# tprelle/janusgraph

Measured on AMD Instinct MI355X. Metric: GTEPS for PageRank iter + BFS, RMAT-24/26, 1/2/4/8 GPUs; % of HBM peak, higher is better.
Workload: dtype f64

## Files before the change

### janusgraph_amd/csrc/jg_api.cpp

```cpp
#include <dlfcn.h>
#include <execinfo.h>

#include <algorithm>
#include <atomic>
#include <cstdlib>
#include <cstring>
#include <limits>
#include <map>
#include <mutex>

#include "jg_cache.h"
#include "jg_internal.h"
#include "jg_labelset.h"

namespace jg {

namespace {
thread_local std::string g_last_error;
}

void rccl_check(ncclResult_t r, const char* what) {
    if (r != ncclSuccess) fail(JG_ERR_RCCL, std::string(what) + ": " + ncclGetErrorString(r));
}

// ... 625 lines not shown
    if (!(cond)) jg::fail(JG_ERR_ARG, msg)

extern "C" {

int jg_abi_version(void) { return JG_ABI_VERSION; }

int jg_tune_set(const char* key, int64_t value) {
    JG_GUARD_BEGIN
    JG_ARG(key, "null key");
    const std::string k(key);
    jg::Tune& t = jg::tune();
    if (k == "dev_poison_probe") {
        jg::dev_poison_probe(value);
        return JG_OK;
    }
    struct Knob {
        const char* name;
        int* field;
        int64_t lo, hi;
    };
    const Knob knobs[] = {
        {"pull_split", &t.pull_split, 0, 1},
        {"halo", &t.halo, 0, 1},
        {"bfs_alpha", &t.bfs_alpha, 1, 1000000},
        {"dobfs_alpha", &t.dobfs_alpha, 1, 1000000},
        {"bfs_beta", &t.bfs_beta, 1, 1000000},
        {"bfs_narrow", &t.bfs_narrow, 0, 1},
        {"nb_alpha", &t.nb_alpha, 1, 1000000},
        {"nb_first", &t.nb_first, 4, 4096},
        {"cc_push", &t.cc_push, 0, 1},
        {"msbfs_sparse", &t.msbfs_sparse, 0, 1},
        {"msbfs_td", &t.msbfs_td, 0, 2},
        {"cc_first", &t.cc_first, 1, 64},
        {"msbfs_skip", &t.msbfs_skip, 0, 1},
        {"msbfs_exit", &t.msbfs_exit, 0, 2},
        {"msbfs_td_rowapply", &t.msbfs_td_rowapply, 0, 1024},
        {"msbfs_td_noprobe", &t.msbfs_td_noprobe, 0, 1000},
        {"msbfs_scan_queue", &t.msbfs_scan_queue, 0, 1001},
        {"msbfs_exit_first", &t.msbfs_exit_first, 1, 256},
        {"msbfs_exit_live", &t.msbfs_exit_live, 0, 1000},
        {"cc_uf", &t.cc_uf, 0, 1},
        {"cc_uf_sharded", &t.cc_uf_sharded, 0, 1},
        {"cc_uf_search", &t.cc_uf_search, 0, 1},
        {"cc_sparse", &t.cc_sparse, 0, 1},
        {"msbfs_split", &t.msbfs_split, 0, 1},
        {"sharded_bfs", &t.sharded_bfs, 0, 1},
        {"bfs_td_split", &t.bfs_td_split, 0, 2},
        {"bfs_td_split_levels", &t.bfs_td_split_levels, 0, 0xffff},
        {"bfs_batch0", &t.bfs_batch0, 1, 64},
        {"bfs_grid_mult", &t.bfs_grid_mult, 1, 64},
        {"bfs_grid", &t.bfs_grid, 64, 65536},
        {"bfs_tail_grid", &t.bfs_tail_grid, 0, 65536},
        {"merge_temporal", &t.merge_temporal, 0, 2},
        {"sd_delta", &t.sd_delta, -1, 1 << 30},
        {"sd_dist32", &t.sd_dist32, 0, 2},
    };
    for (const Knob& kn : knobs) {
        if (k != kn.name) continue;
        if (value < kn.lo || value > kn.hi)
            jg::fail(JG_ERR_ARG, k + " must be in [" + std::to_string(kn.lo) + ", " + std::to_string(kn.hi) + "]");
        *kn.field = (int)value;
        return JG_OK;
    }
    if (k.rfind("band", 0) == 0 && k.size() == 9 && k[4] >= '0' && k[4] <= '3' &&
        (k.substr(5) == "_deg" || k.substr(5) == "_bit" || k.substr(5) == "_sub")) {
        const int i = k[4] - '0';
        if (k.substr(5) == "_deg") {
            JG_ARG(value >= -1, "band degree must be >= 0 (0: unused) or -1 (automatic)");
            t.band_deg[i] = value;
        } else if (k.substr(5) == "_bit") {
            JG_ARG(value == 0 || (value >= 3 && value <= 8), "band bits must be 0 (automatic) or in [3, 8]");
            t.band_bits[i] = value == 0 ? -1 : (int)value;
        } else {
            JG_ARG(value >= 1 && value <= 256 && (value & (value - 1)) == 0, "band sub-slices must be a power of two in [1, 256]");
            int b = 0;
            while ((1 << b) < value) ++b;
            t.band_bits[i] = b;
        }
    } else if (k.size() == 12 && k.compare(0, 11, "merge_stage") == 0 && k[11] >= '0' && k[11] <= '3') {
        JG_ARG(value == -1 || value == 0 || value == 64 || value == 128 || value == 256 || value == 512,
               "merge_stage<i> must be -1 (automatic), 0, 64, 128, 256 or 512");
        t.merge_stage[k[11] - '0'] = (int)value;
    } else if (k == "bfs_td_split_min" || k == "bfs_td_split_max") {
        JG_ARG(value >= 1 && value <= INT32_MAX, "bfs_td_split_min / _max must be in [1, 2^31)");
        (k == "bfs_td_split_min" ? t.bfs_td_split_min : t.bfs_td_split_max) = value;
    } else if (k == "merge_pack") {
        JG_ARG(value == 0 || value == 1 || value == 24, "merge_pack must be 0 (32 bits), 1 (automatic) or 24 (at least 24)");
        t.merge_pack = (int)value;
    } else if (k == "pull_unroll" || k == "pull_nt" || k == "pull_lds" || k == "light_lds" || k == "slice_lds" ||
               k == "pull_short" || k == "pull_overlap" || k == "bfs_persistent") {
    } else {
        jg::fail(JG_ERR_ARG, "unknown tuning key: " + k);
    }
    JG_GUARD_END
}

const char* jg_last_error(void) { return jg::g_last_error.c_str(); }

int jg_comm_unique_id(void* out) {
    JG_GUARD_BEGIN
    JG_ARG(out, "null output");
    ncclUniqueId id;
    jg::rccl_check(ncclGetUniqueId(&id), "ncclGetUniqueId");
    static_assert(sizeof(ncclUniqueId) == JG_UNIQUE_ID_BYTES, "unique id size");
    std::memcpy(out, &id, sizeof id);
    JG_GUARD_END
// ... 834 lines not shown
```

### janusgraph_amd/csrc/jg_internal.h

```cpp
#pragma once

#include <algorithm>
#include <memory>
#include <atomic>
#include <mutex>
#include <functional>
#include <vector>

#include "jg_common.h"
#include "janusgpu.h"

#include <rccl/rccl.h>

namespace jg {

struct Csr {
    int64_t rows = 0;
    int64_t nnz = 0;
    DevBuf<int64_t> row_ptr;
    DevBuf<int32_t> col;
    DevBuf<int32_t> weight;
    mutable int64_t empty_from = -1;
    mutable DevBuf<int32_t> first_col;
    mutable long long wstat[4] = {0, 0, 0, 0};
// ... 68 lines not shown
    return (x ^ (x >> 8) ^ (x >> 16) ^ (x >> 24)) & 255u;
}
__host__ __device__ __forceinline__ uint32_t brev_bits(uint32_t v, int bits) {
    uint32_t r = 0;
    for (int i = 0; i < bits; ++i) r |= ((v >> i) & 1u) << (bits - 1 - i);
    return r;
}
__host__ __device__ __forceinline__ uint32_t sub_key(int64_t c) { return brev_bits(sub_hash(c), 8); }
__host__ __device__ __forceinline__ int sub_slice(int64_t c, int bits) { return (int)(sub_hash(c) & ((1u << bits) - 1)); }

struct Ctx;

struct CompactMap {
    const uint32_t* bits = nullptr;
    const int64_t* off = nullptr;
    const int64_t* qbase = nullptr;
    int64_t S = 0;
    int r = 0, tbits = 31;
    __host__ __device__ bool on() const { return bits != nullptr; }
    __device__ __forceinline__ int32_t operator()(int64_t g) const {
        const int64_t q = g / S, l = g - q * S;
        if (q == r) return (int32_t)l;
        const uint32_t w = bits[g >> 5];
        const int64_t rank = off[g >> 5] + __popc(w & ((1u << (g & 31)) - 1u)) - qbase[q];
        return (int32_t)(((q < r ? q + 1 : q) << tbits) + rank);
    }
};

struct Halo {
    bool on = false;
    int tbits = 31;
    int64_t C = 0;
    DevBuf<uint32_t> bits;
    DevBuf<int64_t> off, qbase;
    DevBuf<int32_t> send_src;
    std::vector<int64_t> send_off, recv_off;
    DevBuf<uint64_t> send_buf;
    int seg_of(int q, int r) const { return q < r ? q + 1 : q; }
    CompactMap map(int64_t S, int r) const {
        CompactMap m;
        if (on) { m.bits = bits.get(); m.off = off.get(); m.qbase = qbase.get(); m.S = S; m.r = r; m.tbits = tbits; }
        return m;
    }
};

struct alignas(16) IdSlot {
    unsigned long long key;
    uint32_t val, pad;
};

struct VecPos {
    int64_t base = 0;
    __device__ __forceinline__ int64_t operator()(int64_t row) const { return base + row; }
};

struct Shard {
    int device = 0;
    int index = 0;
    int vtag = -1;
    hipStream_t stream = nullptr;
    ncclComm_t comm = nullptr;
    int64_t rows = 0;
    Csr in, out, both;
    PullPlan plan_in, plan_both;
    PullPlan plan_out;
    bool plan_out_built = false;
    Halo halo_in, halo_both;
    DevBuf<int32_t> out_degree;
    mutable std::vector<int32_t> dense_of_local_host;
    mutable std::mutex lazy_mu;
    const std::vector<int32_t>& dense_of_local() const;
    DevBuf<int32_t> dense_rows;

    DevBuf<double> pr_contrib[2];
    DevBuf<double> pr_rank;
    DevBuf<double> pr_hub_partial;
    DevBuf<double> pr_split_partial;
    DevBuf<int32_t> cc_split_partial;
    DevBuf<int32_t> cc_msg[2];
    DevBuf<int32_t> cc_label;
    DevBuf<int32_t> cc_rank0;
    DevBuf<int32_t> cc_depth;
    DevBuf<unsigned long long> cc_linked;
    int64_t cc_heavy = -1;
    DevBuf<int32_t> cc_hub_partial;
    DevBuf<int32_t> cc_changed;
    DevBuf<int32_t> bfs_queue[2];
    DevBuf<int64_t> bfs_qoff[2];
    DevBuf<unsigned long long> bfs_bm[2];
    DevBuf<uint8_t> bfs_seen;
    DevBuf<int32_t> bfs_owner;
    DevBuf<unsigned long long> bfs_ctr;
    DevBuf<unsigned char> bfs_state;
    DevBuf<int32_t> bfs_depth;
    bool bfs_depth_tail_clean = false;
    DevBuf<uint8_t> sbfs_stamp;
    DevBuf<uint8_t> sbfs_dirty;
    DevBuf<unsigned long long> sbfs_bq;
    DevBuf<int32_t> sbfs_bpre;
    bool sbfs_stamp_clean = false;
    int bfs_hist[4] = {0, 0, 0, 0};
    int bfs_hist_n = 0;
    int sd_hist[4] = {0, 0, 0, 0};
    int sd_hist_n = 0;
    DevBuf<int32_t> kept_depth;
    DevBuf<int32_t> dag_vertex, dag_depth, dag_pred;
    DevBuf<int64_t> dag_off;
    DevBuf<int64_t> census_vid, census_pop;
    std::vector<DevBuf<uint8_t>> nb_level;
    DevBuf<uint8_t> nb_vis;
    DevBuf<unsigned long long> nb_rest;
    DevBuf<int32_t> nb_queue[2];
    DevBuf<int64_t> nb_qoff[2];
    DevBuf<unsigned long long> nb_ctr;
    DevBuf<unsigned char> nb_state;
    DevBuf<const uint8_t*> nb_table;

    std::vector<hipEvent_t> prof_events;
    std::vector<hipEvent_t> exch_events;
    std::vector<int> prof_units;
};

inline bool same_device(const Shard& sh, int dev) { return sh.device == dev && sh.vtag <= 0; }

struct Graph {
    Ctx* ctx = nullptr;
    int64_t n = 0;
    int P = 1;
    int64_t S = 0;
    uint32_t flags = 0;
    std::vector<std::unique_ptr<Shard>> shards;
    DevBuf<IdSlot> id_table;
    int id_dev = 0;
    std::vector<int64_t> vid;
    DevBuf<int32_t> padded_dev;
    mutable std::vector<int32_t> padded_host;
    mutable std::mutex lazy_mu;
    const std::vector<int32_t>& padded_of_dense() const;
    jg_graph_info info{};
    bool has_weights = false;
    int kept_nsrc = 0;
    int kept_dir = 0;
    int64_t dag_nv = -1, dag_ne = 0;
    int64_t census_listed = -1;
    int64_t top_listed = -1;
    std::vector<int64_t> top_index;
    std::vector<double> top_rank, top_edges;
    bool cc_ranks = false;
    DevBuf<int64_t> cc_vor;
    mutable std::vector<int64_t> cc_vor_host;
    const std::vector<int64_t>& vid_of_rank() const;
    int pr_cur = 0;
    bool pr_begun = false;
    double pr_damping = 0.85;
    int64_t pr_vertex_count = 1;
    int pr_steps = 0;

    int64_t vid_of(int64_t dense) const { return vid.empty() ? dense : vid[dense]; }
    int64_t padded_len() const { return (int64_t)P * S; }
    const Halo& halo(const Shard& sh, uint32_t adj) const { return adj == JG_ADJ_BOTH ? sh.halo_both : sh.halo_in; }
    int64_t vec_len(const Shard& sh, uint32_t adj) const {
        const Halo& h = halo(sh, adj);
        return h.on ? std::max<int64_t>(h.C, 1) : padded_len();
    }
    VecPos vec_pos(const Shard& sh, uint32_t adj) const {
        VecPos p;
        p.base = halo(sh, adj).on ? 0 : (int64_t)sh.index * S;
        return p;
    }
};

struct Ctx {
    std::vector<int> devices;
    int nranks = 1;
    int rank = 0;
    bool logical = false;
    bool vdev = false;
    std::vector<ncclComm_t> comms;
    bool host_transport = false;
    jg_transport transport{};
    std::vector<hipStream_t> streams;
    bool profiling = false;
    jg_stats last{};
    std::atomic<int> live{0};
    int total_shards() const { return nranks * (int)devices.size(); }
};

struct DenseEdges {
    std::vector<int32_t*> src, dst;
    std::vector<int32_t*> weight;
    int64_t m = 0;
    bool capped = false, in_from_in = false;
    std::vector<int32_t*> out_src, in_src, in_dst;
    int64_t m_in = 0;
    int64_t truncated_rows = 0;
};
void build_graph_from_dense(Graph& g, DenseEdges& e);
void generate_rmat_device(int scale, uint64_t seed, int64_t m, int32_t* src, int32_t* dst, hipStream_t s);
void remap_ids_device(const int64_t* d_vid, int64_t n, const int64_t* d_src, const int64_t* d_dst, int64_t m,
                      int32_t* dsrc, int32_t* ddst, hipStream_t s, DevBuf<IdSlot>* table = nullptr);
void dense_of_vids(const Graph& g, const int64_t* vids, int64_t k, int64_t* out, int64_t* padded = nullptr);
void mask_ids_device(const int64_t* masked, const int32_t* dense, int64_t m, int32_t* out, hipStream_t s);
void build_pull_plan(Shard& sh, const Csr& csr, PullPlan& plan, int64_t col_space, int64_t vec_entries,
                     int elem_bytes);
int auto_band_bits(int64_t vec_entries, int elem_bytes);

void rccl_check(ncclResult_t r, const char* what);

void exchange_vec(Graph& g, uint32_t adj, std::vector<void*>& bufs, size_t elem_bytes, ncclDataType_t type);
// ... 156 lines not shown
};
NarrowRun narrow_bfs(Ctx& ctx, Shard& sh, const Csr& push, const Csr& pull, const int64_t* src, int ns, int max_depth,
                     int32_t* planes);
void combine_run(Graph& g, int direction, int combiner, int wrap32, const int64_t* init, int steps, int64_t* out,
                 uint8_t* received_out);

int allreduce_or(Graph& g, int flag);
void allreduce_sum_i64(Graph& g, int64_t* vals, int n);
uint64_t allreduce_or_u64(Graph& g, uint64_t v);

bool pull_split_launches();
bool debug_plan();
bool debug_bfs();

struct Tune {
    int pull_split = 1;
    int64_t band_deg[4] = {96, -1, -1, 0};
    int band_bits[4] = {-1, -1, -1, 3};
    int halo = 1;
    int bfs_alpha = 14;
    int dobfs_alpha = 30;
    int bfs_beta = 24;
    int bfs_narrow = 1;
    int nb_alpha = 30;
    int nb_first = 16;
    int cc_push = 1;
    int msbfs_sparse = 1;
    int msbfs_td = 1;
    int cc_first = 1;
    int msbfs_skip = 1;
    int msbfs_exit = 1;
    int msbfs_td_rowapply = 4;
    int msbfs_td_noprobe = 2;
    int msbfs_scan_queue = 50;
    int msbfs_exit_first = 16;
    int msbfs_exit_live = 950;
    int cc_uf = 1;
    int cc_uf_sharded = 1;
    int cc_uf_search = 1;
    int cc_sparse = 1;
    int msbfs_split = 1;
    int sharded_bfs = 1;
    int bfs_td_split = 2;
    int bfs_td_split_levels = 2;
    int64_t bfs_td_split_min = 65536;
    int64_t bfs_td_split_max = 1 << 20;
    int bfs_batch0 = 10;
    int bfs_grid_mult = 4;
    int bfs_grid = 8192;
    int bfs_tail_grid = 64;
    int sd_dist32 = 1;
    int sd_delta = -1;
    int merge_temporal = 1;
    int merge_stage[4] = {-1, -1, -1, -1};
    int merge_pack = 1;
};
Tune& tune();
void host_allgather(Ctx& c, const void* in, void* out, size_t bytes);
void host_exchange(Ctx& c, const std::vector<int>& speer, const std::vector<const void*>& sbuf,
                   const std::vector<size_t>& sbytes, const std::vector<int>& rpeer, const std::vector<void*>& rbuf,
                   const std::vector<size_t>& rbytes);
int device_cu_count();

bool prof_enabled(const Ctx& c);
void prof_record_start(Ctx& c, Shard& sh);
void prof_record_stop(Ctx& c, Shard& sh, int units = 1);
void prof_collect(Ctx& c, Graph& g);
void exch_record(Ctx& c, Shard& sh);
void prof_discard_exchanges(Graph& g);
struct ExchTimer {
    Graph& g;
    explicit ExchTimer(Graph& gr);
    ~ExchTimer();
};

}

struct jg_ctx {
    jg::Ctx impl;
};
struct jg_graph {
    jg::Graph impl;
    explicit jg_graph(jg::Ctx* c) {
        impl.ctx = c;
        c->live.fetch_add(1);
    }
    ~jg_graph() { impl.ctx->live.fetch_sub(1); }
    jg_graph(const jg_graph&) = delete;
    jg_graph& operator=(const jg_graph&) = delete;
};
```

### janusgraph_amd/csrc/jg_pagerank.hip

```cpp
#include <cstdlib>

#include "jg_pull.h"
#include "jg_scatter.h"

namespace jg {

namespace {

struct PrOp {
    using T = double;
    const double* __restrict__ x;
    double* __restrict__ contrib_out;
    double* __restrict__ rank;
    const int32_t* __restrict__ outdeg;
    VecPos pos;
    double damping, teleport;
    bool write_rank;
    __device__ __forceinline__ double identity() const { return 0.0; }
    __device__ __forceinline__ double combine(double a, double b) const { return __dadd_rn(a, b); }
    __device__ __forceinline__ double gather(int32_t c) const { return x[c]; }
    __device__ __forceinline__ const double* vec() const { return x; }
    __device__ __forceinline__ double shfl_xor(double v, int o) const { return __shfl_xor(v, o, kWave); }
    __device__ __forceinline__ bool active(int64_t) const { return true; }
    __device__ __forceinline__ void finalize(int64_t row, double s) const {
        const double r = __dadd_rn(__dmul_rn(damping, s), teleport);
        if (write_rank) rank[row] = r;
        contrib_out[pos(row)] = r / (double)outdeg[row];
    }
};

__global__ void pr_init_kernel(const int32_t* __restrict__ outdeg, int64_t rows, VecPos pos, double initial,
                               double* __restrict__ contrib, double* __restrict__ rank) {
    for (int64_t l = (int64_t)blockIdx.x * blockDim.x + threadIdx.x; l < rows; l += (int64_t)gridDim.x * blockDim.x) {
        rank[l] = initial;
        contrib[pos(l)] = initial / (double)outdeg[l];
    }
}

void exchange_contrib(Graph& g, int which) {
    std::vector<void*> bufs;
    for (auto& sp : g.shards) bufs.push_back(sp->pr_contrib[which].peer());
    exchange_vec(g, JG_ADJ_IN, bufs, sizeof(double), ncclFloat64);
}

}

void pagerank_begin(Graph& g, double damping, int64_t vertex_count) {
    if (!(g.flags & JG_ADJ_IN)) fail(JG_ERR_UNSUPPORTED, "PageRank needs a graph built with JG_ADJ_IN");
    if (vertex_count == 0) fail(JG_ERR_ARG, "vertexCount must be non-zero");
    for (auto& sp : g.shards) {
        Shard& sh = *sp;
        DeviceGuard dg(sh);
        const int64_t len = g.vec_len(sh, JG_ADJ_IN);
        for (int k = 0; k < 2; ++k) {
            if (sh.pr_contrib[k].size() != (size_t)len) sh.pr_contrib[k].alloc(len);
            JG_HIP(hipMemsetAsync(sh.pr_contrib[k].get(), 0, sh.pr_contrib[k].bytes(), sh.stream));
        }
        if (sh.pr_rank.size() != (size_t)std::max<int64_t>(sh.rows, 1)) {
            const char* f = std::getenv("JG_VDEV_FAULT");
            if (f && *f && *f != '0' && sh.index > 0) {
                DeviceGuard d0(*g.shards[0]);
                sh.pr_rank.alloc(std::max<int64_t>(sh.rows, 1));
            } else {
                sh.pr_rank.alloc(std::max<int64_t>(sh.rows, 1));
            }
        }
        if (sh.pr_hub_partial.size() != (size_t)std::max<int64_t>(sh.plan_in.num_chunks, 1))
            sh.pr_hub_partial.alloc(std::max<int64_t>(sh.plan_in.num_chunks, 1));
        if (sh.pr_split_partial.size() != (size_t)sh.plan_in.split_partial_len()) {
            sh.pr_split_partial.alloc(sh.plan_in.split_partial_len());
        }
        const double initial = 1.0 / (double)vertex_count;
        if (sh.rows > 0) {
            pr_init_kernel<<<grid_for(sh.rows), kBlock, 0, sh.stream>>>(sh.out_degree.get(), sh.rows,
                                                                        g.vec_pos(sh, JG_ADJ_IN), initial,
                                                                        sh.pr_contrib[0].get(), sh.pr_rank.get());
            JG_LAUNCH_CHECK();
        }
    }
    exchange_contrib(g, 0);
    g.pr_cur = 0;
    g.pr_begun = true;
    g.pr_damping = damping;
    g.pr_vertex_count = vertex_count;
    g.pr_steps = 0;
}

void pagerank_steps(Graph& g, int nsteps) {
    if (!g.pr_begun) fail(JG_ERR_STATE, "jg_pagerank_step before jg_pagerank_begin");
    const double teleport = (1.0 - g.pr_damping) / (double)g.pr_vertex_count;
    Ctx* pc = g.ctx->profiling ? g.ctx : nullptr;
    Shard* whole = (pc && g.shards.size() == 1 && g.ctx->total_shards() == 1 && nsteps > 0) ? g.shards[0].get() : nullptr;
    if (whole) {
        DeviceGuard dg(whole->device);
        prof_record_start(*pc, *whole);
        pc = nullptr;
    }
    for (int t = 0; t < nsteps; ++t) {
        const int cur = g.pr_cur, nxt = cur ^ 1;
        for (auto& sp : g.shards) {
            Shard& sh = *sp;
            DeviceGuard dg(sh);
            PrOp op;
            op.x = sh.pr_contrib[cur].get();
            op.contrib_out = sh.pr_contrib[nxt].get();
            op.rank = sh.pr_rank.get();
            op.outdeg = sh.out_degree.get();
            op.pos = g.vec_pos(sh, JG_ADJ_IN);
            op.damping = g.pr_damping;
            op.teleport = teleport;
            op.write_rank = t == nsteps - 1 || g.pr_steps < 2;
            const bool skip_empty = g.pr_steps >= 2;
            launch_pull(sh.in, sh.plan_in, op, sh.pr_hub_partial.get(), sh.stream, pc, &sh, sh.pr_split_partial.get(),
                        skip_empty);
        }
        exchange_contrib(g, nxt);
        g.pr_cur = nxt;
        ++g.pr_steps;
    }
    if (whole) {
        DeviceGuard dg(whole->device);
        prof_record_stop(*g.ctx, *whole, nsteps);
    }
}

void pagerank_end(Graph& g, double* rank_out, double* edge_count_out) {
    if (!g.pr_begun) fail(JG_ERR_STATE, "jg_pagerank_end before jg_pagerank_begin");
    for (auto& sp : g.shards) {
        Shard& sh = *sp;
        DeviceGuard dg(sh);
        JG_HIP(hipStreamSynchronize(sh.stream));
        if (sh.rows == 0) continue;
        if (rank_out) rows_to_dense(g, sh, sh.pr_rank.get(), rank_out);
        if (edge_count_out) rows_to_dense(g, sh, sh.out_degree.get(), edge_count_out);
    }
    prof_collect(*g.ctx, g);
}

}
```

### janusgraph_amd/csrc/jg_pull.h

```cpp
#pragma once

#include <type_traits>

#include "jg_internal.h"
#include "jg_prim.h"

namespace jg {

struct PullArgs {
    const int64_t* __restrict__ row_ptr;
    const int32_t* __restrict__ col;
    const int64_t* __restrict__ chunk_row;
    const int64_t* __restrict__ chunk_begin;
    const int64_t* __restrict__ chunk_end;
    const int64_t* __restrict__ hub_chunk_ptr;
    int64_t num_chunks;
    int64_t num_hub_rows;
    int64_t class_row_begin[kNumClasses];
    int64_t class_row_end[kNumClasses];
    int64_t class_block_begin[kNumClasses + 1];
    int64_t block_offset;
    int64_t skip_rows;
    int runs;
    int64_t run_begin[kRunMax + 1];
// ... 177 lines not shown
            T t = red[0];
#pragma unroll
            for (int w = 1; w < kBlock / kWave; ++w) t = op.combine(t, red[w]);
            hub_partial[b] = t;
        }
        return;
    }
    pull_block_rows<Op, U>(a, op, GlobalGather<Op>{op}, b, (int)threadIdx.x);
}

template <class Op, int U>
__global__ __launch_bounds__(kBlock) void pull_kernel(PullArgs a, Op op, typename Op::T* __restrict__ hub_partial) {
    pull_block<Op, U>(a, op, hub_partial, (int64_t)blockIdx.x + a.block_offset);
}

template <class Op>
__global__ void pull_hub_finalize_kernel(PullArgs a, Op op, const typename Op::T* __restrict__ hub_partial) {
    using T = typename Op::T;
    for (int64_t h = (int64_t)blockIdx.x * blockDim.x + threadIdx.x; h < a.num_hub_rows;
         h += (int64_t)gridDim.x * blockDim.x) {
        const int64_t c0 = a.hub_chunk_ptr[h], c1 = a.hub_chunk_ptr[h + 1];
        if (a.chunk_row[c0] < a.skip_rows) continue;
        T acc = op.identity();
        for (int64_t k = c0; k < c1; ++k) acc = op.combine(acc, hub_partial[k]);
        op.finalize(a.chunk_row[c0], acc);
    }
}

constexpr int kMergeThreads = 1024;
constexpr int kMergeWaves = kMergeThreads / kWave;
constexpr int kMergeEpl = kMergeTask / kWave;
constexpr int kMergeLdsBytes = 160 * 1024;

struct MergeArgs {
    const uint4* __restrict__ pack_a;
    const uint32_t* __restrict__ pack_b;
    const uint8_t* __restrict__ heads;
    const int32_t* __restrict__ meta;
    const int64_t* __restrict__ sub_begin;
    const int64_t* __restrict__ sub_end;
    const int64_t* __restrict__ sub_base;
    int64_t tasks;
    int bits;
    int stage;
    const uint32_t* __restrict__ live;
};

struct HotSegs {
    int32_t hs = 0;
    int tbits = 31;
    int nseg = 1;
};

template <class Op, bool MSEG = true>
struct SliceGather {
    using T = typename Op::T;
    const Op& op;
    lds_ptr<const T> lds;
    uint32_t hg;
    int sb;
    int bits;
    uint32_t hmask, h;
    uint32_t idcell;
    __device__ __forceinline__ bool is_hot(uint32_t loc) const {
        if constexpr (!MSEG) return loc < (hg << 4);
        return ((loc >> 4) & ((1u << sb) - 1u)) < hg;
    }
    __device__ __forceinline__ T hot(uint32_t loc, bool valid) const {
        if constexpr (!MSEG) return lds[valid && loc < (hg << 4) ? loc : idcell];
        const uint32_t g = loc >> 4, j = g & ((1u << sb) - 1u), seg = g >> sb;
        return lds[valid && j < hg ? (((seg * hg + j) << 4) | (loc & 15u)) : idcell];
    }
    __device__ __forceinline__ int32_t col(uint32_t loc) const {
        const uint32_t x = (loc >> 4) << bits;
        const uint32_t hx = (x ^ (x >> 8) ^ (x >> 16) ^ (x >> 24)) & hmask;
        return (int32_t)(((x | (h ^ hx)) << 4) | (loc & 15u));
    }
    __device__ __forceinline__ T cold(uint32_t loc, bool valid, bool lds_on) const {
        T v = op.identity();
        if (valid && !(lds_on && is_hot(loc))) v = op.gather(col(loc));
        return v;
    }
};

template <int W>
__device__ __forceinline__ uint32_t unpack_entry(const uint32_t (&d)[W / 4], int u) {
    const int o = W * u, i = o >> 5, sh = o & 31;
    uint32_t v = d[i] >> sh;
    if (sh + W > 32) v |= d[i + 1] << (32 - sh);
    if constexpr (W < 32) v &= (1u << W) - 1u;
    return v;
}

template <class T>
__device__ __forceinline__ T lane_up(T v, int lane, int d) {
    static_assert(sizeof(T) % 4 == 0, "whole dwords");
    int w[sizeof(T) / 4];
    __builtin_memcpy(w, &v, sizeof(T));
    const int addr = ((lane - d) & (kWave - 1)) << 2;
#pragma unroll
    for (size_t i = 0; i < sizeof(T) / 4; ++i) w[i] = __builtin_amdgcn_ds_bpermute(addr, w[i]);
    __builtin_memcpy(&v, w, sizeof(T));
    return v;
}

template <class Op, class = void>
struct op_task_live : std::false_type {};
template <class Op>
struct op_task_live<Op, std::void_t<decltype(Op::kTaskLive)>> : std::bool_constant<Op::kTaskLive> {};

template <class Op, bool LDS, int PW, bool MSEG = false>
__global__ __launch_bounds__(kMergeThreads) void pull_merge_kernel(MergeArgs a, Op op, typename Op::T* __restrict__ partial,
                                                                   typename Op::T* __restrict__ carry, HotSegs hs,
                                                                   int temporal) {
    using T = typename Op::T;
    extern __shared__ __align__(16) unsigned char merge_lds[];
    const int S = 1 << a.bits;
    const int xs = S < kXcds ? S : kXcds;
    const int rep = kXcds / xs;
    const int per = S / xs;
    const int w = (int)(blockIdx.x >> 3), W = (int)(gridDim.x >> 3);
    const int xcd = (int)(blockIdx.x & (kXcds - 1));
    const int wave = threadIdx.x / kWave, lane = threadIdx.x % kWave;
    lds_ptr<T> hotv = (lds_ptr<T>)merge_lds;
    const int gshift = 4 + a.bits;
    const int hg = hs.hs >> gshift;
    const int nl = hs.nseg * hg;
    lds_ptr<T> stg = hotv + (nl * 16 + 1) + wave * (a.stage + 1);
    lds_ptr<uint32_t> tctr = (lds_ptr<uint32_t>)(hotv + (nl * 16 + 1) + kMergeWaves * (a.stage + 1));
    const int rounds = temporal ? per : 1;
    const uint32_t hmask = (1u << a.bits) - 1u;
    auto image_line = [&](int seg, int j, int hh) {
        const int64_t grp = ((int64_t)seg << (hs.tbits - gshift)) + j;
        return (grp << a.bits) + (int64_t)(hh ^ (sub_hash(grp << gshift) & hmask));
    };
    for (int rd = 0; rd < rounds; ++rd) {
    const int h = (xcd % xs) | ((temporal ? rd : w % per) << 3);
    const int64_t g = (int64_t)(temporal ? w : w / per) * rep + xcd / xs;
    const int64_t G = (int64_t)(temporal ? W : W / per) * rep;
    if constexpr (LDS) {
        if (rd > 0) __syncthreads();
        constexpr int kStage = 8;
        constexpr int kUnit = 16 / (int)sizeof(T);
        static_assert(16 % sizeof(T) == 0 && kUnit <= 16, "16-byte staging units");
        const unsigned char* src = reinterpret_cast<const unsigned char*>(op.vec());
        const int units = nl * 16 / kUnit;
        using u4 = uint32_t __attribute__((ext_vector_type(4)));
        lds_ptr<u4> hv4 = (lds_ptr<u4>)merge_lds;
        for (int q0 = 0; q0 < units; q0 += kStage * kMergeThreads) {
            u4 buf[kStage];
#pragma unroll
            for (int u = 0; u < kStage; ++u) {
                const int q = q0 + u * kMergeThreads + (int)threadIdx.x;
                const int i = q * kUnit, sg = i >> 4;
                int seg = 0, j = sg;
                if (hs.nseg > 1) {
                    seg = sg / hg;
                    j = sg - seg * hg;
                }
                buf[u] = u4{0, 0, 0, 0};
                if (q < units)
                    buf[u] = *reinterpret_cast<const u4*>(src + (image_line(seg, j, h) * 16 + (i & 15)) * (int64_t)sizeof(T));
            }
#pragma unroll
            for (int u = 0; u < kStage; ++u) {
                const int q = q0 + u * kMergeThreads + (int)threadIdx.x;
                if (q < units) hv4[q] = buf[u];
            }
        }
        if (threadIdx.x == 0) {
            hotv[nl * 16] = op.identity();
            *tctr = 0u;
        }
        __syncthreads();
    }
    const SliceGather<Op, MSEG> lg{op,       hotv, (uint32_t)hg, hs.tbits - gshift, a.bits, (1u << a.bits) - 1u, (uint32_t)h,
                             (uint32_t)nl * 16u};
    const int64_t base = a.sub_base[h];
    const int64_t ntask = a.sub_base[h + 1] - base;
    const int64_t hbegin = a.sub_begin[h], hend = a.sub_end[h];
    constexpr bool dyn = LDS;
    const int64_t grot = (g + rd) % G;
    auto task_of = [&](int64_t j) { return j * G + grot; };
    auto grab = [&]() -> int64_t {
        uint32_t j = 0;
        if (lane == 0) j = __hip_atomic_fetch_add(tctr, 1u, __ATOMIC_RELAXED, __HIP_MEMORY_SCOPE_WORKGROUP);
        return task_of((int64_t)__builtin_amdgcn_readfirstlane(j));
    };
    int64_t jstat = wave;
    auto advance = [&]() -> int64_t {
        if (dyn) return grab();
        jstat += kMergeWaves;
        return task_of(jstat);
    };
    auto dead = [&](int64_t kk) -> bool {
        if constexpr (!op_task_live<Op>::value) return false;
        if (a.live == nullptr || kk >= ntask) return false;
        const uint64_t tt = (uint64_t)(base + kk);
        const uint32_t wd = __builtin_amdgcn_readfirstlane(a.live[tt >> 5]);
        return ((wd >> (tt & 31)) & 1u) == 0;
    };
    int64_t k = dyn ? grab() : task_of(jstat);
    while (dead(k)) k = advance();
    if (k >= ntask) continue;
    static_assert(kMergeEpl == 8, "a lane chunk is 8 entries");
    constexpr int DB = PW / 4 - 4;
    auto chunk = [&](int64_t kk) { return (hbegin >> 3) + kk * kWave + lane; };
    auto meta_idx = [&](int64_t kk) { return 2 * (base + kk) + (lane & 1); };
    auto head_idx = [&](int64_t kk) { return (base + kk) * kWave + lane; };
    auto ld = [](const auto* p) { return *p; };
    using v4u = uint32_t __attribute__((ext_vector_type(4)));
    using v2u = uint32_t __attribute__((ext_vector_type(2)));
    auto load_chunk = [&](int64_t kk, uint32_t (&d)[PW / 4]) {
        const int64_t x = chunk(kk);
        const v4u va = ld(reinterpret_cast<const v4u*>(a.pack_a) + x);
        d[0] = va.x, d[1] = va.y, d[2] = va.z, d[3] = va.w;
        if constexpr (DB == 1) {
            d[4] = ld(a.pack_b + x);
        } else if constexpr (DB == 2) {
            const v2u vb = ld(reinterpret_cast<const v2u*>(a.pack_b) + x);
            d[4] = vb.x, d[5] = vb.y;
        } else {
            const v4u vb = ld(reinterpret_cast<const v4u*>(a.pack_b) + x);
            d[4] = vb.x, d[5] = vb.y, d[6] = vb.z, d[7] = vb.w;
        }
    };
    uint32_t cd[PW / 4];
    load_chunk(k, cd);
    uint32_t hb = ld(a.heads + head_idx(k));
    int32_t mw = ld(a.meta + meta_idx(k));
// ... 211 lines not shown
}

template <class Op>
__global__ void pull_slice_finalize_kernel(int64_t row0, int64_t rows, Op op, FinalizeBands fb,
                                           const typename Op::T* __restrict__ partial) {
    for (int64_t r = row0 + (int64_t)blockIdx.x * blockDim.x + threadIdx.x; r < rows; r += (int64_t)gridDim.x * blockDim.x)
        slice_finalize_row(r, op, fb, partial);
}

template <class Op, int U>
__global__ __launch_bounds__(kBlock) void pull_light_finalize_kernel(PullArgs a, Op op,
                                                                     typename Op::T* __restrict__ hub_partial,
                                                                     FinalizeBands fb,
                                                                     const typename Op::T* __restrict__ partial,
                                                                     int64_t split_rows, int64_t fin_blocks,
                                                                     int64_t fin_row0) {
    const int64_t b = blockIdx.x;
    if (b < fin_blocks) {
        const int64_t r = fin_row0 + b * kBlock + threadIdx.x;
        if (r < split_rows) slice_finalize_row<Op>(r, op, fb, partial);
        return;
    }
    pull_block<Op, U>(a, op, hub_partial, b - fin_blocks + a.block_offset);
}


template <class Op>
void launch_pull(const Csr& csr, const PullPlan& plan, const Op& op, typename Op::T* hub_partial, hipStream_t s,
                 Ctx* prof_ctx = nullptr, Shard* prof_shard = nullptr, typename Op::T* split_partial = nullptr,
                 bool skip_empty = false, const uint32_t* const* task_live = nullptr, int64_t caller_rows = 0) {
    using T = typename Op::T;
    const bool split = tune().pull_split && plan.split_rows > 0 && split_partial != nullptr;
    if (task_live != nullptr && !op_task_live<Op>::value)
        fail(JG_ERR_UNSUPPORTED, "launch_pull: this Op does not declare kTaskLive");
    size_t band0 = 0;
    if (caller_rows > 0) {
        while (band0 < plan.bands.size() && plan.bands[band0]->row_end <= caller_rows) ++band0;
        if (!split || band0 == 0 || plan.bands[band0 - 1]->row_end != caller_rows)
            fail(JG_ERR_UNSUPPORTED, "launch_pull: caller rows must end a prefix of the split bands");
    }
    PullArgs a = make_pull_args(csr, plan, split);
    if (skip_empty) a.class_block_begin[kNumClasses] = a.class_block_begin[kZeroClass];
    const int64_t blocks = a.class_block_begin[kNumClasses];
    if (prof_ctx) prof_record_start(*prof_ctx, *prof_shard);
    if (split) {
        static bool attr = false;
        if (!attr) {
            JG_HIP(hipFuncSetAttribute((const void*)pull_merge_kernel<Op, true, 20>,
                                       hipFuncAttributeMaxDynamicSharedMemorySize, kMergeLdsBytes));
            JG_HIP(hipFuncSetAttribute((const void*)pull_merge_kernel<Op, true, 24>,
                                       hipFuncAttributeMaxDynamicSharedMemorySize, kMergeLdsBytes));
            JG_HIP(hipFuncSetAttribute((const void*)pull_merge_kernel<Op, true, 32>,
                                       hipFuncAttributeMaxDynamicSharedMemorySize, kMergeLdsBytes));
            JG_HIP(hipFuncSetAttribute((const void*)pull_merge_kernel<Op, true, 20, true>,
                                       hipFuncAttributeMaxDynamicSharedMemorySize, kMergeLdsBytes));
            JG_HIP(hipFuncSetAttribute((const void*)pull_merge_kernel<Op, true, 24, true>,
                                       hipFuncAttributeMaxDynamicSharedMemorySize, kMergeLdsBytes));
            JG_HIP(hipFuncSetAttribute((const void*)pull_merge_kernel<Op, true, 32, true>,
                                       hipFuncAttributeMaxDynamicSharedMemorySize, kMergeLdsBytes));
            attr = true;
        }
        for (size_t bi = band0; bi < plan.bands.size(); ++bi) {
            const SliceBand& bd = *plan.bands[bi];
            if (bd.tasks == 0) continue;
            int stage = tune().merge_stage[std::min<size_t>(bi, 3)];
            if (stage < 0) {
                const double heads = (double)bd.subrows / (double)std::max<int64_t>(bd.tasks, 1);
                stage = 128;
                while (stage < 4.0 * heads && stage < 256) stage *= 2;
            }
            MergeArgs ma{bd.pack_a.get(), bd.pack_b.get(), bd.heads.get(), bd.meta.get(), bd.sub_begin.get(),
                         bd.sub_end.get(), bd.sub_base.get(), bd.tasks, bd.bits, stage,
                         task_live ? task_live[bi] : nullptr};
            T* part = split_partial + bd.part_off;
            T* carry = split_partial + bd.carry_off;
            const int64_t S = 1ll << bd.bits, gsz = 16 * S;
            const unsigned grid = (unsigned)std::max<int64_t>(S, (int64_t)device_cu_count() / S * S);
            const int64_t stage_bytes = (int64_t)kMergeWaves * (stage + 1) * (int64_t)sizeof(T);
            const int64_t hot_max = (int64_t)((kMergeLdsBytes - stage_bytes - 16) / (int64_t)sizeof(T) - 16) * S;
            HotSegs hs;
            hs.tbits = plan.seg_tbits;
            hs.nseg = plan.nseg;
            const int64_t seg_cap = plan.nseg == 1 ? plan.col_space : (1ll << plan.seg_tbits) - gsz;
            hs.hs = plan.lds_ok ? (int32_t)(std::min<int64_t>(hot_max / plan.nseg, seg_cap) / gsz * gsz) : 0;
            const int temporal = tune().merge_temporal == 2 || (tune().merge_temporal == 1 && plan.temporal);
            const size_t lds = hs.hs > 0 ? (size_t)(hs.nseg * (hs.hs / S) + 1) * sizeof(T) + (size_t)stage_bytes + 16 : 0;
            auto go = [&](auto kern) { kern<<<grid, kMergeThreads, lds, s>>>(ma, op, part, carry, hs, temporal); };
            if (hs.hs > 0 && hs.nseg > 1) {
                if (bd.width == 20) go(pull_merge_kernel<Op, true, 20, true>);
                else if (bd.width == 24) go(pull_merge_kernel<Op, true, 24, true>);
                else go(pull_merge_kernel<Op, true, 32, true>);
            } else if (hs.hs > 0) {
                if (bd.width == 20) go(pull_merge_kernel<Op, true, 20>);
                else if (bd.width == 24) go(pull_merge_kernel<Op, true, 24>);
                else go(pull_merge_kernel<Op, true, 32>);
            } else {
                if (bd.width == 20) go(pull_merge_kernel<Op, false, 20>);
                else if (bd.width == 24) go(pull_merge_kernel<Op, false, 24>);
                else go(pull_merge_kernel<Op, false, 32>);
            }
            JG_LAUNCH_CHECK();
        }
        FixupBands fx{};
        for (size_t bi = band0; bi < plan.bands.size(); ++bi) {
            const auto& bp = plan.bands[bi];
            if (fx.n == kMaxBands) fail(JG_ERR_UNSUPPORTED, "too many split bands");
            fx.meta[fx.n] = bp->meta.get();
            fx.part_off[fx.n] = bp->part_off;
            fx.carry_off[fx.n] = bp->carry_off;
            fx.task_begin[fx.n + 1] = fx.task_begin[fx.n] + bp->tasks;
            ++fx.n;
        }
        if (fx.task_begin[fx.n] > 0) {
            pull_merge_fixup_kernel<Op><<<grid_for(fx.task_begin[fx.n], kBlock, 0), kBlock, 0, s>>>(fx, op, split_partial);
            JG_LAUNCH_CHECK();
        }
    }
    auto launch = [&](unsigned grid) {
        pull_kernel<Op, 4><<<grid, kBlock, 0, s>>>(a, op, hub_partial);
        JG_LAUNCH_CHECK();
    };
    FinalizeBands fb{};
    if (split) {
        for (const auto& bp : plan.bands) {
            if (fb.n == kMaxBands) fail(JG_ERR_UNSUPPORTED, "too many split bands");
            fb.sub_word[fb.n] = bp->sub_word.get();
            fb.row_begin[fb.n] = bp->row_begin;
            fb.row_end[fb.n] = bp->row_end;
            fb.part_off[fb.n] = bp->part_off;
            fb.bits[fb.n] = bp->bits;
            ++fb.n;
        }
    }
    const bool fuse = split && !pull_split_launches();
    if (fuse) {
        const int64_t fin_blocks = (plan.split_rows - caller_rows + kBlock - 1) / kBlock;
        const unsigned grid = (unsigned)(fin_blocks + blocks);
        pull_light_finalize_kernel<Op, 4><<<grid, kBlock, 0, s>>>(a, op, hub_partial, fb, split_partial, plan.split_rows,
                                                                  fin_blocks, caller_rows);
        JG_LAUNCH_CHECK();
    } else if (pull_split_launches()) {
// ... 24 lines not shown
```

Measured before the change: 387.9.

## Store PageRank contribution vector in per-slice hashed layout for merge kernels

```diff
diff --git a/janusgraph_amd/csrc/jg_api.cpp b/janusgraph_amd/csrc/jg_api.cpp
--- a/janusgraph_amd/csrc/jg_api.cpp
+++ b/janusgraph_amd/csrc/jg_api.cpp
@@ -701,6 +701,7 @@
         {"bfs_grid", &t.bfs_grid, 64, 65536},
         {"bfs_tail_grid", &t.bfs_tail_grid, 0, 65536},
         {"merge_temporal", &t.merge_temporal, 0, 2},
+        {"pr_sliced_vec", &t.pr_sliced_vec, 0, 1},
         {"sd_delta", &t.sd_delta, -1, 1 << 30},
         {"sd_dist32", &t.sd_dist32, 0, 2},
     };
diff --git a/janusgraph_amd/csrc/jg_internal.h b/janusgraph_amd/csrc/jg_internal.h
--- a/janusgraph_amd/csrc/jg_internal.h
+++ b/janusgraph_amd/csrc/jg_internal.h
@@ -144,6 +144,27 @@
 struct VecPos {
     int64_t base = 0;
     __device__ __forceinline__ int64_t operator()(int64_t row) const { return base + row; }
+};
+
+struct SlicedVec {
+    int bits = -1;
+    uint32_t G = 0;
+    __host__ __device__ bool on() const { return bits >= 0; }
+    __host__ __device__ int64_t slice_len() const { return (int64_t)G * 16; }
+    __host__ __device__ int64_t padded_len() const { return slice_len() << bits; }
+    __host__ __device__ __forceinline__ uint32_t line(uint32_t L) const {
+        const uint32_t h = (L ^ (L >> 8) ^ (L >> 16) ^ (L >> 24)) & ((1u << bits) - 1u);
+        return h * G + (L >> bits);
+    }
+    __host__ __device__ __forceinline__ uint32_t pos(int64_t c) const {
+        return (line((uint32_t)(c >> 4)) << 4) | ((uint32_t)c & 15u);
+    }
+    static SlicedVec make(int bits, int64_t len) {
+        SlicedVec v;
+        v.bits = bits;
+        v.G = (uint32_t)((len + (16ll << bits) - 1) / (16ll << bits));
+        return v;
+    }
 };
 
 struct Shard {
@@ -247,6 +268,7 @@
     double pr_damping = 0.85;
     int64_t pr_vertex_count = 1;
     int pr_steps = 0;
+    SlicedVec pr_sliced;
 
     int64_t vid_of(int64_t dense) const { return vid.empty() ? dense : vid[dense]; }
     int64_t padded_len() const { return (int64_t)P * S; }
@@ -509,6 +531,7 @@
     int sd_dist32 = 1;
     int sd_delta = -1;
     int merge_temporal = 1;
+    int pr_sliced_vec = 1;
     int merge_stage[4] = {-1, -1, -1, -1};
     int merge_pack = 1;
 };
diff --git a/janusgraph_amd/csrc/jg_pagerank.hip b/janusgraph_amd/csrc/jg_pagerank.hip
--- a/janusgraph_amd/csrc/jg_pagerank.hip
+++ b/janusgraph_amd/csrc/jg_pagerank.hip
@@ -7,33 +7,42 @@
 
 namespace {
 
-struct PrOp {
+template <bool SL>
+struct PrOpT {
     using T = double;
+    static constexpr bool kSlicedVec = SL;
     const double* __restrict__ x;
     double* __restrict__ contrib_out;
     double* __restrict__ rank;
     const int32_t* __restrict__ outdeg;
     VecPos pos;
+    SlicedVec sv;
     double damping, teleport;
     bool write_rank;
     __device__ __forceinline__ double identity() const { return 0.0; }
     __device__ __forceinline__ double combine(double a, double b) const { return __dadd_rn(a, b); }
-    __device__ __forceinline__ double gather(int32_t c) const { return x[c]; }
+    __device__ __forceinline__ double gather(int32_t c) const {
+        if constexpr (SL) return x[sv.pos(c)];
+        else return x[c];
+    }
+    __device__ __forceinline__ int64_t vec_line(int64_t L) const { return SL ? (int64_t)sv.line((uint32_t)L) : L; }
+    __device__ __forceinline__ const double* slice(int h) const { return x + (int64_t)h * sv.slice_len(); }
     __device__ __forceinline__ const double* vec() const { return x; }
     __device__ __forceinline__ double shfl_xor(double v, int o) const { return __shfl_xor(v, o, kWave); }
     __device__ __forceinline__ bool active(int64_t) const { return true; }
     __device__ __forceinline__ void finalize(int64_t row, double s) const {
         const double r = __dadd_rn(__dmul_rn(damping, s), teleport);
         if (write_rank) rank[row] = r;
-        contrib_out[pos(row)] = r / (double)outdeg[row];
+        if constexpr (SL) contrib_out[sv.pos(pos(row))] = r / (double)outdeg[row];
+        else contrib_out[pos(row)] = r / (double)outdeg[row];
     }
 };
 
-__global__ void pr_init_kernel(const int32_t* __restrict__ outdeg, int64_t rows, VecPos pos, double initial,
+__global__ void pr_init_kernel(const int32_t* __restrict__ outdeg, int64_t rows, VecPos pos, SlicedVec sv, double initial,
                                double* __restrict__ contrib, double* __restrict__ rank) {
     for (int64_t l = (int64_t)blockIdx.x * blockDim.x + threadIdx.x; l < rows; l += (int64_t)gridDim.x * blockDim.x) {
         rank[l] = initial;
-        contrib[pos(l)] = initial / (double)outdeg[l];
+        contrib[sv.on() ? (int64_t)sv.pos(pos(l)) : pos(l)] = initial / (double)outdeg[l];
     }
 }
 
@@ -43,15 +52,41 @@
     exchange_vec(g, JG_ADJ_IN, bufs, sizeof(double), ncclFloat64);
 }
 
+template <bool SL>
+void pr_superstep(Graph& g, Shard& sh, int cur, double teleport, bool write_rank, Ctx* pc) {
+    PrOpT<SL> op;
+    op.x = sh.pr_contrib[cur].get();
+    op.contrib_out = sh.pr_contrib[cur ^ 1].get();
+    op.rank = sh.pr_rank.get();
+    op.outdeg = sh.out_degree.get();
+    op.pos = g.vec_pos(sh, JG_ADJ_IN);
+    op.sv = g.pr_sliced;
+    op.damping = g.pr_damping;
+    op.teleport = teleport;
+    op.write_rank = write_rank;
+    const bool skip_empty = g.pr_steps >= 2;
+    launch_pull(sh.in, sh.plan_in, op, sh.pr_hub_partial.get(), sh.stream, pc, &sh, sh.pr_split_partial.get(),
+                skip_empty);
+}
+
 }
 
 void pagerank_begin(Graph& g, double damping, int64_t vertex_count) {
     if (!(g.flags & JG_ADJ_IN)) fail(JG_ERR_UNSUPPORTED, "PageRank needs a graph built with JG_ADJ_IN");
     if (vertex_count == 0) fail(JG_ERR_ARG, "vertexCount must be non-zero");
+    g.pr_sliced = SlicedVec{};
+    if (tune().pr_sliced_vec && g.shards.size() == 1 && g.P == 1 && g.ctx->total_shards() == 1) {
+        const Shard& sh = *g.shards[0];
+        const PullPlan& p = sh.plan_in;
+        if (tune().pull_split && p.split_rows > 0 && !p.bands.empty() && p.lds_ok && p.nseg == 1 && !g.halo(sh, JG_ADJ_IN).on) {
+            const SlicedVec sv = SlicedVec::make(p.bands[0]->bits, g.vec_len(sh, JG_ADJ_IN));
+            if (sv.slice_len() < (1ll << 28)) g.pr_sliced = sv;
+        }
+    }
     for (auto& sp : g.shards) {
         Shard& sh = *sp;
         DeviceGuard dg(sh);
-        const int64_t len = g.vec_len(sh, JG_ADJ_IN);
+        const int64_t len = g.pr_sliced.on() ? g.pr_sliced.padded_len() : g.vec_len(sh, JG_ADJ_IN);
         for (int k = 0; k < 2; ++k) {
             if (sh.pr_contrib[k].size() != (size_t)len) sh.pr_contrib[k].alloc(len);
             JG_HIP(hipMemsetAsync(sh.pr_contrib[k].get(), 0, sh.pr_contrib[k].bytes(), sh.stream));
@@ -73,7 +108,7 @@
         const double initial = 1.0 / (double)vertex_count;
         if (sh.rows > 0) {
             pr_init_kernel<<<grid_for(sh.rows), kBlock, 0, sh.stream>>>(sh.out_degree.get(), sh.rows,
-                                                                        g.vec_pos(sh, JG_ADJ_IN), initial,
+                                                                        g.vec_pos(sh, JG_ADJ_IN), g.pr_sliced, initial,
                                                                         sh.pr_contrib[0].get(), sh.pr_rank.get());
             JG_LAUNCH_CHECK();
         }
@@ -101,18 +136,9 @@
         for (auto& sp : g.shards) {
             Shard& sh = *sp;
             DeviceGuard dg(sh);
-            PrOp op;
-            op.x = sh.pr_contrib[cur].get();
-            op.contrib_out = sh.pr_contrib[nxt].get();
-            op.rank = sh.pr_rank.get();
-            op.outdeg = sh.out_degree.get();
-            op.pos = g.vec_pos(sh, JG_ADJ_IN);
-            op.damping = g.pr_damping;
-            op.teleport = teleport;
-            op.write_rank = t == nsteps - 1 || g.pr_steps < 2;
-            const bool skip_empty = g.pr_steps >= 2;
-            launch_pull(sh.in, sh.plan_in, op, sh.pr_hub_partial.get(), sh.stream, pc, &sh, sh.pr_split_partial.get(),
-                        skip_empty);
+            const bool write_rank = t == nsteps - 1 || g.pr_steps < 2;
+            if (g.pr_sliced.on()) pr_superstep<true>(g, sh, cur, teleport, write_rank, pc);
+            else pr_superstep<false>(g, sh, cur, teleport, write_rank, pc);
         }
         exchange_contrib(g, nxt);
         g.pr_cur = nxt;
diff --git a/janusgraph_amd/csrc/jg_pull.h b/janusgraph_amd/csrc/jg_pull.h
--- a/janusgraph_amd/csrc/jg_pull.h
+++ b/janusgraph_amd/csrc/jg_pull.h
@@ -253,7 +253,7 @@
     int nseg = 1;
 };
 
-template <class Op, bool MSEG = true>
+template <class Op, bool MSEG = true, bool SL0 = false>
 struct SliceGather {
     using T = typename Op::T;
     const Op& op;
@@ -263,6 +263,7 @@
     int bits;
     uint32_t hmask, h;
     uint32_t idcell;
+    const T* __restrict__ xb = nullptr;
     __device__ __forceinline__ bool is_hot(uint32_t loc) const {
         if constexpr (!MSEG) return loc < (hg << 4);
         return ((loc >> 4) & ((1u << sb) - 1u)) < hg;
@@ -279,7 +280,12 @@
     }
     __device__ __forceinline__ T cold(uint32_t loc, bool valid, bool lds_on) const {
         T v = op.identity();
-        if (valid && !(lds_on && is_hot(loc))) v = op.gather(col(loc));
+        if constexpr (SL0) {
+            __builtin_assume(loc < (1u << 28));
+            if (valid && !(lds_on && is_hot(loc))) v = xb[loc];
+        } else {
+            if (valid && !(lds_on && is_hot(loc))) v = op.gather(col(loc));
+        }
         return v;
     }
 };
@@ -310,7 +316,12 @@
 template <class Op>
 struct op_task_live<Op, std::void_t<decltype(Op::kTaskLive)>> : std::bool_constant<Op::kTaskLive> {};
 
-template <class Op, bool LDS, int PW, bool MSEG = false>
+template <class Op, class = void>
+struct op_sliced : std::false_type {};
+template <class Op>
+struct op_sliced<Op, std::void_t<decltype(Op::kSlicedVec)>> : std::bool_constant<Op::kSlicedVec> {};
+
+template <class Op, bool LDS, int PW, bool MSEG = false, bool SL0 = false>
 __global__ __launch_bounds__(kMergeThreads) void pull_merge_kernel(MergeArgs a, Op op, typename Op::T* __restrict__ partial,
                                                                    typename Op::T* __restrict__ carry, HotSegs hs,
                                                                    int temporal) {
@@ -335,6 +346,7 @@
         const int64_t grp = ((int64_t)seg << (hs.tbits - gshift)) + j;
         return (grp << a.bits) + (int64_t)(hh ^ (sub_hash(grp << gshift) & hmask));
     };
+    (void)image_line;
     for (int rd = 0; rd < rounds; ++rd) {
     const int h = (xcd % xs) | ((temporal ? rd : w % per) << 3);
     const int64_t g = (int64_t)(temporal ? w : w / per) * rep + xcd / xs;
@@ -345,6 +357,7 @@
         constexpr int kUnit = 16 / (int)sizeof(T);
         static_assert(16 % sizeof(T) == 0 && kUnit <= 16, "16-byte staging units");
         const unsigned char* src = reinterpret_cast<const unsigned char*>(op.vec());
+        if constexpr (SL0) src = reinterpret_cast<const unsigned char*>(op.slice(h));
         const int units = nl * 16 / kUnit;
         using u4 = uint32_t __attribute__((ext_vector_type(4)));
         lds_ptr<u4> hv4 = (lds_ptr<u4>)merge_lds;
@@ -353,13 +366,23 @@
 #pragma unroll
             for (int u = 0; u < kStage; ++u) {
                 const int q = q0 + u * kMergeThreads + (int)threadIdx.x;
+                buf[u] = u4{0, 0, 0, 0};
+                if constexpr (SL0) {
+                    if (q < units) buf[u] = *reinterpret_cast<const u4*>(src + (int64_t)q * 16);
+                    continue;
+                }
                 const int i = q * kUnit, sg = i >> 4;
                 int seg = 0, j = sg;
                 if (hs.nseg > 1) {
                     seg = sg / hg;
                     j = sg - seg * hg;
                 }
-                buf[u] = u4{0, 0, 0, 0};
+                if constexpr (op_sliced<Op>::value) {
+                    if (q < units)
+                        buf[u] = *reinterpret_cast<const u4*>(
+                            src + (op.vec_line(image_line(seg, j, h)) * 16 + (i & 15)) * (int64_t)sizeof(T));
+                    continue;
+                }
                 if (q < units)
                     buf[u] = *reinterpret_cast<const u4*>(src + (image_line(seg, j, h) * 16 + (i & 15)) * (int64_t)sizeof(T));
             }
@@ -375,8 +398,10 @@
         }
         __syncthreads();
     }
-    const SliceGather<Op, MSEG> lg{op,       hotv, (uint32_t)hg, hs.tbits - gshift, a.bits, (1u << a.bits) - 1u, (uint32_t)h,
-                             (uint32_t)nl * 16u};
+    const T* xb = nullptr;
+    if constexpr (SL0) xb = op.slice(h);
+    const SliceGather<Op, MSEG, SL0> lg{op,       hotv, (uint32_t)hg, hs.tbits - gshift, a.bits, (1u << a.bits) - 1u, (uint32_t)h,
+                                        (uint32_t)nl * 16u, xb};
     const int64_t base = a.sub_base[h];
     const int64_t ntask = a.sub_base[h + 1] - base;
     const int64_t hbegin = a.sub_begin[h], hend = a.sub_end[h];
@@ -694,12 +719,21 @@
                                        hipFuncAttributeMaxDynamicSharedMemorySize, kMergeLdsBytes));
             JG_HIP(hipFuncSetAttribute((const void*)pull_merge_kernel<Op, true, 32>,
                                        hipFuncAttributeMaxDynamicSharedMemorySize, kMergeLdsBytes));
-            JG_HIP(hipFuncSetAttribute((const void*)pull_merge_kernel<Op, true, 20, true>,
-                                       hipFuncAttributeMaxDynamicSharedMemorySize, kMergeLdsBytes));
-            JG_HIP(hipFuncSetAttribute((const void*)pull_merge_kernel<Op, true, 24, true>,
-                                       hipFuncAttributeMaxDynamicSharedMemorySize, kMergeLdsBytes));
-            JG_HIP(hipFuncSetAttribute((const void*)pull_merge_kernel<Op, true, 32, true>,
-                                       hipFuncAttributeMaxDynamicSharedMemorySize, kMergeLdsBytes));
+            if constexpr (op_sliced<Op>::value) {
+                JG_HIP(hipFuncSetAttribute((const void*)pull_merge_kernel<Op, true, 20, false, true>,
+                                           hipFuncAttributeMaxDynamicSharedMemorySize, kMergeLdsBytes));
+                JG_HIP(hipFuncSetAttribute((const void*)pull_merge_kernel<Op, true, 24, false, true>,
+                                           hipFuncAttributeMaxDynamicSharedMemorySize, kMergeLdsBytes));
+                JG_HIP(hipFuncSetAttribute((const void*)pull_merge_kernel<Op, true, 32, false, true>,
+                                           hipFuncAttributeMaxDynamicSharedMemorySize, kMergeLdsBytes));
+            } else {
+                JG_HIP(hipFuncSetAttribute((const void*)pull_merge_kernel<Op, true, 20, true>,
+                                           hipFuncAttributeMaxDynamicSharedMemorySize, kMergeLdsBytes));
+                JG_HIP(hipFuncSetAttribute((const void*)pull_merge_kernel<Op, true, 24, true>,
+                                           hipFuncAttributeMaxDynamicSharedMemorySize, kMergeLdsBytes));
+                JG_HIP(hipFuncSetAttribute((const void*)pull_merge_kernel<Op, true, 32, true>,
+                                           hipFuncAttributeMaxDynamicSharedMemorySize, kMergeLdsBytes));
+            }
             attr = true;
         }
         for (size_t bi = band0; bi < plan.bands.size(); ++bi) {
@@ -728,7 +762,28 @@
             const int temporal = tune().merge_temporal == 2 || (tune().merge_temporal == 1 && plan.temporal);
             const size_t lds = hs.hs > 0 ? (size_t)(hs.nseg * (hs.hs / S) + 1) * sizeof(T) + (size_t)stage_bytes + 16 : 0;
             auto go = [&](auto kern) { kern<<<grid, kMergeThreads, lds, s>>>(ma, op, part, carry, hs, temporal); };
-            if (hs.hs > 0 && hs.nseg > 1) {
+            if constexpr (op_sliced<Op>::value) {
+                if (hs.nseg > 1) fail(JG_ERR_UNSUPPORTED, "launch_pull: a sliced vector has one segment");
+                if (bd.bits != op.sv.bits) {
+                    if (hs.hs > 0) {
+                        if (bd.width == 20) go(pull_merge_kernel<Op, true, 20>);
+                        else if (bd.width == 24) go(pull_merge_kernel<Op, true, 24>);
+                        else go(pull_merge_kernel<Op, true, 32>);
+                    } else {
+                        if (bd.width == 20) go(pull_merge_kernel<Op, false, 20>);
+                        else if (bd.width == 24) go(pull_merge_kernel<Op, false, 24>);
+                        else go(pull_merge_kernel<Op, false, 32>);
+                    }
+                } else if (hs.hs > 0) {
+                    if (bd.width == 20) go(pull_merge_kernel<Op, true, 20, false, true>);
+                    else if (bd.width == 24) go(pull_merge_kernel<Op, true, 24, false, true>);
+                    else go(pull_merge_kernel<Op, true, 32, false, true>);
+                } else {
+                    if (bd.width == 20) go(pull_merge_kernel<Op, false, 20, false, true>);
+                    else if (bd.width == 24) go(pull_merge_kernel<Op, false, 24, false, true>);
+                    else go(pull_merge_kernel<Op, false, 32, false, true>);
+                }
+            } else if (hs.hs > 0 && hs.nseg > 1) {
                 if (bd.width == 20) go(pull_merge_kernel<Op, true, 20, true>);
                 else if (bd.width == 24) go(pull_merge_kernel<Op, true, 24, true>);
                 else go(pull_merge_kernel<Op, true, 32, true>);
```

Result: no change. 390.4, median of 6 (+0.6%).
